# Xinjie-Q/Boosting-NeRV

Hardware: AMD Instinct MI355X
Metric: train frames/sec (higher is better)
Workload: dtype fp32; 1 GPU; NeRV-boost 1.5M (1489577 params, fc_dim 30) train step on a synthetic Bunny-shaped clip 132x3x720x1280: decoder fwd + Fusion10_freq + bwd + fused Adan; frames resident in HBM; global_batch=1, per_gpu_batch=1, parallelism=dp1, hipgraph=True, rccl_ranks=0, collective_in_graph=False

## Files before the change

boosting_nerv_amd/_lib.py:

```python
import ctypes as C
import os

import torch

_HERE = os.path.dirname(os.path.abspath(__file__))
LIB_PATH = os.environ.get("BNERV_LIB") or os.path.join(_HERE, "libbnerv_hip.so")

MAX_DENSE_GROUPS = 40
ADAN_MAX_TENSORS = 48
SFT_CHUNKS = 32
LOSS_STATS = 5
DENSE_DX_CHUNK = 64

ACT_NONE, ACT_RELU, ACT_SIN = 0, 1, 2
IN_PLAIN, IN_AFFINE, IN_GELU_AFFINE, IN_UNSHUFFLE, IN_TANHGRAD = 0, 1, 2, 3, 4
EP_BIAS, EP_BIAS_SIN, EP_BIAS_RES, EP_BIAS_TANH, EP_PLAIN, EP_DGELU, EP_DSIN, EP_BIAS_GELU, EP_DGELU_SAVED = 0, 1, 2, 3, 4, 5, 6, 7, 8
CONV_FAM = ("head1_fwd", "head1_dgrad", "head3", "stem_dgrad", "small", "small96", "wide_bf16", "q4", "generic")
WGRAD_FAM = ("stem", "gemm1x1", "lean", "wide_bf16", "wide_f32", "generic")
PAIR_FORM = ("stem", "q4_lean", "small_wide", "bf16_wide", "head")

_fp = C.c_void_p


class DenseFwdDesc(C.Structure):
# ... 83 lines not shown
    "bnerv_abi_version": (_I, []),
    "bnerv_last_error": (C.c_char_p, []),
    "bnerv_build_arch": (C.c_char_p, []),
    "bnerv_pe_fwd_f32": (_I, [_V, _V, _V, _V, _I, _I]),
    "bnerv_pe_fwd_f64": (_I, [_V, _V, _V, _V, _I, _I]),
    "bnerv_pe_fwd_f32_from_f64": (_I, [_V, _V, _V, _V, _I, _I]),
    "bnerv_dense_grouped_fwd": (_I, [_V, C.POINTER(DenseFwdDesc), _I, _I]),
    "bnerv_time_branch_fwd": (_I, [_V, C.POINTER(TimeBranchDesc), C.POINTER(TimeBranchMlp)]),
    "bnerv_dense_grouped_bwd": (_I, [_V, C.POINTER(DenseBwdDesc), _I, _I]),
    "bnerv_sft_affine_fwd": (_I, [_V, _V, _V, _V, _V, _I, _I, _I]),
    "bnerv_sft_affine_bwd": (_I, [_V, _V, _V, _V, _V, _V, _I, _I, _I]),
    "bnerv_reduce_slabs": (_I, [_V, _V, _I, _I, _V]),
    "bnerv_ctx_create": (_I, [C.POINTER(C.c_void_p)]),
    "bnerv_ctx_destroy": (None, [_V]),
    "bnerv_ctx_scratch_bytes": (_Z, [_V]),
    "bnerv_ctx_reserve": (_I, [_V, _Z]),
    "bnerv_ctx_wplan_record": (_I, [_V]),
    "bnerv_ctx_wplan_freeze": (_I, [_V]),
    "bnerv_ctx_wplan_run": (_I, [_V, _V]),
    "bnerv_ctx_wplan_run_fetch": (_I, [_V, _V, _V, _V, _V, _I, _Z, _V, _V]),
    "bnerv_ctx_wplan_end": (_I, [_V]),
    "bnerv_ctx_wplan_entries": (_I, [_V]),
    "bnerv_reduce_slabs_deferred": (_I, [_V, _V, _V, _I, _I, _V]),
    "bnerv_flush_deferred": (_I, [_V, _V]),
    "bnerv_deferred_pending": (_I, [_V]),
    "bnerv_conv_tiles": (_I, [_I, _I]),
    "bnerv_conv_igemm": (_I, [_V, C.POINTER(ConvDesc)]),
    "bnerv_conv_splitk_ws_bytes": (_Z, [C.POINTER(ConvDesc)]),
    "bnerv_conv_partial_rows": (_I, [C.POINTER(ConvDesc)]),
    "bnerv_conv_family": (_I, [C.POINTER(ConvDesc), C.POINTER(C.c_int)]),
    "bnerv_conv_wgrad_ws_bytes": (_Z, [_I, _I, _I, _I, _I, _I]),
    "bnerv_conv_wgrad_pair": (_I, [_V, C.POINTER(ConvDesc), C.POINTER(WgradDesc)]),
    "bnerv_conv_wgrad_pair_form": (_I, [C.POINTER(ConvDesc), C.POINTER(WgradDesc), C.POINTER(C.c_int)]),
    "bnerv_conv_wgrad": (_I, [_V, C.POINTER(WgradDesc)]),
    "bnerv_conv_wgrad_family": (_I, [C.POINTER(WgradDesc), C.POINTER(C.c_int)]),
    "bnerv_conv5_ws_bytes": (_Z, [_I, _I]),
    "bnerv_conv5_igemm": (_I, [_V, C.POINTER(ConvDesc), _V, _Z]),
    "bnerv_conv5_wgrad_ws_bytes": (_Z, [_I, _I, _I, _I, _I]),
    "bnerv_conv5_wgrad": (_I, [_V, C.POINTER(WgradDesc)]),
    "bnerv_gelu_fwd": (_I, [_V, _V, _V, _V, _Z]),
    "bnerv_mul": (_I, [_V, _V, _V, _V, _Z]),
    "bnerv_cem_ws_bytes": (_Z, [_I, _I]),
    "bnerv_cem_scale_fwd": (_I, [_V, C.POINTER(CemChunk), _V, _V, _Z]),
    "bnerv_cem_scale_bwd": (_I, [_V, C.POINTER(CemChunkBwd), _V, _V, _V, _V, _Z]),
    "bnerv_dense_gemm_fwd": (_I, [_V, _V, _V, _V, _V, _V, _I, _I, _I, _I]),
    "bnerv_dense_gemm_bwd_ws_bytes": (_Z, [_I, _I, _I]),
    "bnerv_dense_gemm_bwd": (_I, [_V, _V, _V, _V, _V, _V, _V, _V, _V, _V, _Z, _I, _I, _I, _I]),
    "bnerv_cnx_mlp_fwd": (_I, [_V, _V, _V, _V, _V, _V, _V, _V, _V, _V, _I, _I, _I]),
    "bnerv_cnx_mlp_bwd": (_I, [_V, _V, _V, _V, _V, _V, _V, _V, _V, _I, _I, _I]),
    "bnerv_cnx_param_grads": (_I, [_V, _V, _V, _V, _V, _V, _V, _V, _V, _I]),
    "bnerv_ans_encode_gaussian": (C.c_long, [_V, _Z, _I, _I, C.c_double, C.c_double, _V, _Z]),
    "bnerv_ans_decode_gaussian": (_I, [_V, _Z, _Z, _I, _I, C.c_double, C.c_double, _V]),
    "bnerv_ans_encode_categorical": (C.c_long, [_V, _Z, _V, _I, _V, _Z]),
    "bnerv_ans_decode_categorical": (_I, [_V, _Z, _Z, _V, _I, _V]),
    "bnerv_dwconv_fwd": (_I, [_V, _V, _V, _V, _V, _I, _I, _I, _I, _I, _I]),
    "bnerv_dwconv_wgrad_ws_bytes": (_Z, [_I, _I, _I, _I, _I]),
    "bnerv_dwconv_wgrad": (_I, [_V, _V, _V, _V, _V, _Z, _I, _I, _I, _I, _I, _V]),
    "bnerv_lncf_fwd": (_I, [_V, _V, _V, _V, _V, _I, _I, _I, _F]),
    "bnerv_lncf_bwd_ws_bytes": (_Z, [_I, _I, _I]),
    "bnerv_lncf_bwd": (_I, [_V, _V, _V, _V, _V, _V, _V, _Z, _I, _I, _I, _F]),
    "bnerv_loss_ws_bytes": (_Z, [_I, _I, _I, _I, _I, _I]),
    "bnerv_fft_prepare": (_I, [_I, _I]),
    "bnerv_loss_fwd_bwd": (_I, [_V, C.POINTER(LossDesc)]),
    "bnerv_msssim": (_I, [_V, _V, _V, _V, _V, _Z, _I, _I, _I, _I]),
    "bnerv_loss_ssim_ws_bytes": (_Z, [_I, _I, _I, _I, _I]),
    "bnerv_loss_ssim_prepare": (_I, [_I, _I]),
# ... 158 lines not shown
```

boosting_nerv_amd/csrc/abi.hip:

```cpp
#include "common.h"
#include <string.h>

namespace { thread_local char g_err[512] = ""; }

int bnerv_set_error(int code, const char* fmt, ...) {
    va_list ap;
    va_start(ap, fmt);
    vsnprintf(g_err, sizeof(g_err), fmt, ap);
    va_end(ap);
    return code;
}

extern "C" int bnerv_abi_version(void) { return BNERV_ABI_VERSION; }
extern "C" const char* bnerv_last_error(void) { return g_err; }
extern "C" const char* bnerv_build_arch(void) { return "gfx950"; }

#include "sidejob.h"
#include <new>
#include <vector>

namespace {
__global__ __launch_bounds__(256) void side_flush_kernel(const SidePack sp) {
    __shared__ float red[256];
    side_slice<SidePack, true>(sp, blockIdx.x, red);
// ... 19 lines not shown
    j.slices = (count + j.epb - 1) / j.epb;
    return j;
}
}

void bnerv_side_push(bnerv_ctx* ctx, hipStream_t st, const void* src, int n_slabs, int count, int ncols, float* out, float* out2, const float* fold_scale, const float* fold_shift) {
    const SideJob j = make_job(src, n_slabs, count, ncols, out, out2, fold_scale, fold_shift);
    if (ctx) { ctx->queue.push_back(j); return; }
    SidePack sp;
    sp.j[0] = j;
    sp.n_jobs = 1;
    sp.n_slices = j.slices;
    hipLaunchKernelGGL(side_flush_kernel, dim3(sp.n_slices), dim3(256), 0, st, sp);
}

void bnerv_side_take(bnerv_ctx* ctx, SidePack* sp, int max_slices) {
    sp->n_jobs = 0;
    sp->n_slices = 0;
    if (!ctx) return;
    std::vector<SideJob>& q = ctx->queue;
    int n = 0;
    size_t i = 0;
    while (i < q.size() && n < SIDE_MAX_JOBS) {
        if (q[i].fs) { ++i; continue; }
        if (sp->n_slices + q[i].slices > max_slices) break;
        sp->j[n] = q[i];
        sp->n_slices += q[i].slices;
        ++n;
        q.erase(q.begin() + (long)i);
    }
    sp->n_jobs = n;
}

int bnerv_side_pending(const bnerv_ctx* ctx) { return ctx ? (int)ctx->queue.size() : 0; }

int bnerv_side_flush(bnerv_ctx* ctx, hipStream_t st) {
    while (ctx && !ctx->queue.empty()) {
        SideFlushPack sp;
        std::vector<SideJob>& q = ctx->queue;
        int n = 0;
        sp.n_slices = 0;
        while (n < (int)q.size() && n < SIDE_FLUSH_JOBS) {
            sp.j[n] = q[n];
            sp.start[n] = sp.n_slices;
            sp.n_slices += q[n].slices;
            ++n;
        }
        for (int k = n; k < SIDE_FLUSH_JOBS; ++k) sp.start[k] = 0x7fffffff;
        sp.n_jobs = n;
        q.erase(q.begin(), q.begin() + n);
        hipLaunchKernelGGL(side_flush_many_kernel, dim3(sp.n_slices), dim3(256), 0, st, sp);
        BNERV_LAUNCH_CHECK("side_flush");
    }
    return BNERV_OK;
}

extern "C" int bnerv_ctx_create(bnerv_ctx** out) {
    BNERV_REQUIRE(out != nullptr, "ctx_create: null output");
    *out = new (std::nothrow) bnerv_ctx();
    return *out ? BNERV_OK : bnerv_set_error(BNERV_E_ARG, "ctx_create: out of memory");
}
extern "C" void bnerv_ctx_destroy(bnerv_ctx* ctx) {
    if (ctx && ctx->scratch) (void)hipFree(ctx->scratch);
    if (ctx) bnerv_wplan_free(ctx);
    delete ctx;
}

extern "C" size_t bnerv_ctx_scratch_bytes(const bnerv_ctx* ctx) { return ctx ? ctx->scratch_bytes : 0; }

// ... 36 lines not shown
```

boosting_nerv_amd/csrc/sidejob.h:

```cpp
#pragma once
#include "common.h"

constexpr int SIDE_MAX_JOBS = 4;

struct SideJob {
    const float* src;
    float* out;
    float* out2;
    int n_slabs, count, ncols;
    int epb;
    int slices;
    const float* fs;
    const float* ft;
};

struct SidePack {
    SideJob j[SIDE_MAX_JOBS];
    int n_jobs, n_slices;
};
constexpr int SIDE_FLUSH_JOBS = 32;
struct SideFlushPack {
    SideJob j[SIDE_FLUSH_JOBS];
    int n_jobs, n_slices;
    int start[SIDE_FLUSH_JOBS];
};

#include <vector>
struct bnerv_ctx {
    std::vector<SideJob> queue;
    void* scratch = nullptr;
    size_t scratch_bytes = 0;
    struct BfWPlan* wplan = nullptr;
};
void bnerv_wplan_free(bnerv_ctx* ctx);
void* bnerv_ctx_scratch(bnerv_ctx* ctx, size_t bytes, hipStream_t st);

void bnerv_side_push(bnerv_ctx* ctx, hipStream_t st, const void* src, int n_slabs, int count, int ncols, float* out, float* out2,
                     const float* fold_scale = nullptr, const float* fold_shift = nullptr);
void bnerv_side_take(bnerv_ctx* ctx, SidePack* sp, int max_slices);
int bnerv_side_flush(bnerv_ctx* ctx, hipStream_t st);
int bnerv_side_pending(const bnerv_ctx* ctx);

template <class Pack>
__device__ __forceinline__ int side_find_job(const Pack& sp, int* s) {
    int j = 0;
    while (j < sp.n_jobs - 1 && *s >= sp.j[j].slices) { *s -= sp.j[j].slices; ++j; }
    return j;
}
template <>
__device__ __forceinline__ int side_find_job<SideFlushPack>(const SideFlushPack& sp, int* s) {
    const int k = (int)(threadIdx.x & 63);
    const int st = k < sp.n_jobs ? sp.start[k < SIDE_FLUSH_JOBS ? k : 0] : 0x7fffffff;
    const unsigned long long m = __ballot(st <= *s);
    const int j = __popcll(m) - 1;
    *s -= __shfl(st, j, 64);
    return __builtin_amdgcn_readfirstlane(j);
}

template <class Pack, bool FOLD = false>
__device__ __forceinline__ void side_slice(const Pack& sp, int s, float* red) {
    const int j = side_find_job(sp, &s);
    const SideJob& job = sp.j[j];
    const int epb = job.epb, lanes = 256 / epb;
    const int e = threadIdx.x % epb, lane = threadIdx.x / epb;
    const int i = s * epb + e;
    const bool fold = FOLD && job.fs != nullptr;
    float acc = 0.f, acc2 = 0.f;
    int fci = 0;
    bool fbias = false;
    if (i < job.count) {
        size_t cnt = (size_t)job.count;
        size_t i0 = (size_t)i, i1 = 0;
        if (fold) {
            const int co = i / job.ncols, n = i - co * job.ncols, rowl = job.ncols + 8;
// ... 58 lines not shown
```

boosting_nerv_amd/csrc/wgrad.hip:

```cpp
#include "common.h"
#include "sidejob.h"
#include "split16.h"
#include "conv4_body.h"
#include "convs_body.h"
#if defined(BNERV_TRACE) || defined(BNERV_TRACE_BW)
static __device__ unsigned long long g_trace_w[1024 * 4 * 8 * 8];
#endif
#ifdef BNERV_TRACE_BW
#define BTRACE(it_, slot) do { if (lane == 0 && blockIdx.x < 1024 && (unsigned)(it_) < 8u) g_trace_w[((blockIdx.x * 4 + wave) * 8 + (it_)) * 8 + (slot)] = __builtin_amdgcn_s_memtime(); } while (0)
#endif
#include "wgrad_bfw_body.h"
#include "route.h"
bool bnerv_stem_wgrad_ok(const bnerv_wgrad_desc& d);
int bnerv_stem_wgrad_launch(hipStream_t st, const bnerv_wgrad_desc& d);
bool bnerv_stem_pair_ok(const bnerv_conv_desc& c, const bnerv_wgrad_desc& d);
int bnerv_stem_pair_launch(hipStream_t st, const bnerv_conv_desc& c, const bnerv_wgrad_desc& d);
int bnerv_wgrad1x1_slabs(const bnerv_wgrad_desc& d);
int bnerv_wgrad1x1_launch(hipStream_t st, const bnerv_wgrad_desc& d);

namespace {
using namespace bnerv_wb;

constexpr int TH = 8, TW = 32;
constexpr int CSG = TH * TW + 2;
// ... 1335 lines not shown
    const bool red_ep = c.ep_mode == BNERV_EP_DGELU_SAVED || c.ep_mode == BNERV_EP_DSIN;
    const int fused_min = fused_env >= 0 ? fused_env : (red_ep ? 1024 : 0);
    if (fused_min > 0 && total_items >= fused_min && total_items >= 8 && c.x == w.g && c.Cin == w.Cout && c.Cout == w.Cin && c.B == w.B &&
        w.g_s == 1 && (w.g_mode == BNERV_IN_PLAIN || w.g_mode == BNERV_IN_UNSHUFFLE)) {
        p.kind = Q4P_SHARED;
        p.grid = p.n_w = total_items < 512 ? (total_items & ~7) : 512;
        const float* raw_aux = c.ep_mode == BNERV_EP_DSIN ? c.aux0 : c.aux1;
        if (red_ep && w.in_mode == BNERV_IN_AFFINE && !switch_off("BNERV_PAIR_FOLD") && c.B == 1 && raw_aux == w.x && w.scale && w.shift && aligned16(w.x) &&
            (size_t)p.grid * w.Cout * (ncols + 8) * sizeof(float) <= w.ws_bytes)
            p.kind = Q4P_FOLD;
        return p;
    }
    p.kind = Q4P_INTERLEAVED;
    p.n_conv = total_items < 768 ? total_items : 768;
    p.n_conv = (p.n_conv + 7) & ~7;
    p.n_w = wlean_blocks(w);
    p.grid = p.n_conv + p.n_w;
    if (total_items >= 2 * PAIR_MIX && p.n_w >= PAIR_MIX) {
        p.n_w = PAIR_MIX; p.n_conv = -PAIR_MIX; p.grid = 2 * PAIR_MIX;
    }
    return p;
}

template <class F>
int q4_pair_modes(const bnerv_conv_desc& c, const bnerv_wgrad_desc& w, F&& f) {
#define BNERV_PAIR_CASE(E, I) if (c.ep_mode == E && w.in_mode == I) return f(mode_c<E>{}, mode_c<I>{});
    BNERV_PAIR_CASE(BNERV_EP_DGELU_SAVED, BNERV_IN_AFFINE)
    BNERV_PAIR_CASE(BNERV_EP_DSIN, BNERV_IN_AFFINE)
    BNERV_PAIR_CASE(BNERV_EP_PLAIN, BNERV_IN_PLAIN)
#undef BNERV_PAIR_CASE
    return -1;
}

template <int EP, int WIN>
int launch_pair(hipStream_t st, bnerv_conv::KArgs& ka, const WArgs& wa, const Q4PairPlan& p) {
    bnerv_q4::q4_prepare(ka);
    SidePack side;
    if (p.kind == Q4P_FOLD) {
        if constexpr ((EP == BNERV_EP_DGELU_SAVED || EP == BNERV_EP_DSIN) && WIN == BNERV_IN_AFFINE) {
            const size_t ldsf = pair_fused_lds_bytes();
            if (const int rc = dyn_lds<&pair_fused_kernel<EP, WIN>>(ldsf, "pair_fused")) return rc;
            const size_t ldsd = pair_fold_lds_bytes();
            if (const int rc = dyn_lds<&pair_fold_kernel<EP>>(ldsd, "pair_fold")) return rc;
            bnerv_side_take(wa.d.ctx, &side, 2 * p.n_w);
            hipLaunchKernelGGL((pair_fold_kernel<EP>), dim3(p.grid), dim3(256), ldsd, st, ka, wa, side);
            BNERV_LAUNCH_CHECK("pair_fold");
            return BNERV_OK;
        }
    }
    if (p.kind != Q4P_INTERLEAVED) {
        const size_t ldsf = pair_fused_lds_bytes();
        if (const int rc = dyn_lds<&pair_fused_kernel<EP, WIN>>(ldsf, "pair_fused")) return rc;
        bnerv_side_take(wa.d.ctx, &side, 2 * p.n_w);
        hipLaunchKernelGGL((pair_fused_kernel<EP, WIN>), dim3(p.grid), dim3(256), ldsf, st, ka, wa, side);
        BNERV_LAUNCH_CHECK("pair_fused");
        return BNERV_OK;
    }
    const int n_grows = wa.d.Cout <= 12 ? 12 : 16;
    size_t lds = bnerv_q4::q4_lds_bytes();
    const size_t lw = wlean_lds_bytes<3>(n_grows);
    if (lw > lds) lds = lw;
    if (const int rc = dyn_lds<&conv_wgrad_pair_kernel<EP, WIN>>(lds, "conv_wgrad_pair")) return rc;
    bnerv_side_take(wa.d.ctx, &side, 2 * p.n_w);
    hipLaunchKernelGGL((conv_wgrad_pair_kernel<EP, WIN>), dim3(p.grid), dim3(256), lds, st, ka, wa, n_grows, p.n_conv, side, PAIR_PAT);
    BNERV_LAUNCH_CHECK("conv_wgrad_pair");
    return BNERV_OK;
}

struct WideRoleArgs { int slots, ngn, ngm; };
template <int IN, int GM2, int MTW, int NTW>
struct WideRole {
    static __device__ __forceinline__ void run(const WArgs& wa, const WideRoleArgs& r, const SidePack& side, int vb, int vgrid) { wgrad_wide_body<IN, GM2, MTW, NTW>(wa, r.slots, side, vb, vgrid); }
    static size_t lds(const WArgs& wa) { return wgrad_wide_lds_bytes<MTW, NTW>(wa.d.Cout); }
};
template <int IN, int SP, int MTW, int GM2>
struct BfwRole {
    static __device__ __forceinline__ void run(const WArgs& wa, const WideRoleArgs& r, const SidePack& side, int vb, int vgrid) { wgrad_bfw_body<IN, SP, MTW, GM2>(wa, r.slots, r.ngn, r.ngm, side, vb, vgrid); }
    static size_t lds(const WArgs&) { return wgrad_bfw_lds_bytes<SP, MTW>(); }
};
template <class WR, int CIN, int CEP, int CNQ>
__global__ __launch_bounds__(256, 2) void small_pair_kernel(const bnerv_convs::SArgs sa, const WArgs wa, const WideRoleArgs r, const int n_c, const int n_c8,
                                                            const int c_tiles, const int c_groups, const SidePack side) {
    const int b = (int)blockIdx.x;
    if (b < n_c8) {
        if (b >= n_c) return;
        const int q = b / c_tiles;
        bnerv_convs::conv_small_body<CIN, CEP, CNQ>(sa, b - q * c_tiles, q % c_groups, q / c_groups);
    } else {
        WR::run(wa, r, side, b - n_c8, (int)gridDim.x - n_c8);
    }
}
template <class WR, int CIN, int CEP, int CNQ>
int launch_small_pair(hipStream_t st, const bnerv_convs::SArgs& sa, const WArgs& wa, const WideRoleArgs& r, int n_w) {
    size_t lds = bnerv_convs::convs_lds_bytes<CNQ>();
    const size_t lw = WR::lds(wa);
    if (lw > lds) lds = lw;
    if (const int rc = dyn_lds<&small_pair_kernel<WR, CIN, CEP, CNQ>>(lds, "small_pair")) return rc;
    const int c_tiles = sa.tiles_x * sa.tiles_y, c_groups = cdiv(sa.d.Cout, 16);
    const int n_c = c_tiles * c_groups * sa.d.B, n_c8 = (n_c + 7) & ~7;
    SidePack side;
    bnerv_side_take(wa.d.ctx, &side, 2 * n_w);
    hipLaunchKernelGGL((small_pair_kernel<WR, CIN, CEP, CNQ>), dim3(n_c8 + n_w), dim3(256), lds, st, sa, wa, r, n_c, n_c8, c_tiles, c_groups, side);
    BNERV_LAUNCH_CHECK("small_pair");
    return BNERV_OK;
}

template <class T> struct type_c { using type = T; };
template <class F>
int small_pair_modes(const bnerv_conv_desc& c, const bnerv_wgrad_desc& w, const WRoute& wr, F&& f) {
    const int cnq = bnerv_convs_nq(c);
    const bool up = w.g_s == 2 && w.in_mode == BNERV_IN_PLAIN && w.g_mode == BNERV_IN_UNSHUFFLE;
    const bool tat = w.g_s == 1 && w.in_mode == BNERV_IN_AFFINE && w.g_mode != BNERV_IN_TANHGRAD;
#define BNERV_SP(WR, I, E, Q) if (c.in_mode == I && c.ep_mode == E && cnq == Q) return f(type_c<WR>{}, mode_c<I>{}, mode_c<E>{}, mode_c<Q>{});
    if (wr.family == BNERV_WGRAD_FAM_WIDE_BF16 && split_wide_mode() == (int)SP_BF16X6) {
        if (up && wr.bw.mtw == 2) { using WR = BfwRole<BNERV_IN_PLAIN, SP_BF16X6, 2, 1>; BNERV_SP(WR, BNERV_IN_UNSHUFFLE, BNERV_EP_PLAIN, 8) BNERV_SP(WR, BNERV_IN_UNSHUFFLE, BNERV_EP_PLAIN, 16) }
        if (up && wr.bw.mtw == 3) { using WR = BfwRole<BNERV_IN_PLAIN, SP_BF16X6, 3, 1>; BNERV_SP(WR, BNERV_IN_UNSHUFFLE, BNERV_EP_PLAIN, 16) }
        if (tat && wr.bw.mtw == 2) { using WR = BfwRole<BNERV_IN_AFFINE, SP_BF16X6, 2, 0>; BNERV_SP(WR, BNERV_IN_PLAIN, BNERV_EP_DGELU_SAVED, 8) BNERV_SP(WR, BNERV_IN_PLAIN, BNERV_EP_DSIN, 8) }
    }
    if (wr.family == BNERV_WGRAD_FAM_WIDE_F32 && wr.wide.mtw == 1 && wr.wide.ntw == 8 && tat) {
        using WR = WideRole<BNERV_IN_AFFINE, 0, 1, 8>;
        BNERV_SP(WR, BNERV_IN_PLAIN, BNERV_EP_DGELU_SAVED, 4) BNERV_SP(WR, BNERV_IN_PLAIN, BNERV_EP_DSIN, 4)
    }
#undef BNERV_SP
    return -1;
}

bool small_pair_ok(const bnerv_conv_desc& c, int cvec, const bnerv_wgrad_desc& w, const WRoute& wr) {
    if (!bnerv_convs_ok(c, cvec) || bnerv_convs_nq(c) == 24) return false;
    if (c.ep_mode == BNERV_EP_PLAIN && bnerv_conv_splitk_ws_bytes(&c) != 0) return false;
    if (!(w.k == 3 && w.B == c.B && w.H == c.H && w.W == c.W && w.defer_finish && w.ctx && w.ctx == c.ctx)) return false;
    return small_pair_modes(c, w, wr, [](auto...) { return 0; }) == 0;
}

int small_pair_launch(hipStream_t st, const bnerv_conv_desc& c, const WArgs& wa, const WRoute& wr) {
    const bnerv_convs::SArgs sa = bnerv_convs_sargs(c);
    const bool bf = wr.family == BNERV_WGRAD_FAM_WIDE_BF16;
    const WideRoleArgs r = bf ? WideRoleArgs{wr.bw.slots, wr.bw.ngroups_n, wr.bw.ngroups_m} : WideRoleArgs{wr.wide.slots, 0, 0};
    const int n_w = bf ? 8 * wr.bw.slots * wr.bw.ngroups_n * wr.bw.ngroups_m : 8 * wr.wide.slots * wr.wide.ngroups * wr.wide.mgroups;
    return small_pair_modes(c, wa.d, wr, [&](auto role, auto in, auto ep, auto nq) {
        return launch_small_pair<typename decltype(role)::type, decltype(in)::value, decltype(ep)::value, decltype(nq)::value>(st, sa, wa, r, n_w);
    });
}
}

constexpr int HB_KMAX = 4, HB_CMAX = 16;
struct HeadBwdArgs { const float* g; const float* img; const float* x; const float* w; float* dx; float* slab; int B, K, C, transposed; size_t HW; int nq; };
template <int K, int C>
__global__ __launch_bounds__(256) void head1x1_bwd_kernel(const HeadBwdArgs a) {
    __shared__ float s_w[HB_KMAX * HB_CMAX];
    __shared__ float s_red[4][HB_KMAX * (HB_CMAX + 1)];
    const int tid = threadIdx.x, lane = tid & 63, wave = tid >> 6;
    if (tid < K * C) {
        const int k = tid / C, c = tid - k * C;
        s_w[k * HB_CMAX + c] = a.transposed ? a.w[k * C + c] : a.w[c * K + k];
    }
    if (lane < K * (C + 1)) s_red[wave][(lane / (C + 1)) * (HB_CMAX + 1) + lane % (C + 1)] = 0.f;
    __syncthreads();
    const int total = a.B * a.nq;
    const int rounds = (total + (int)gridDim.x * 256 - 1) / ((int)gridDim.x * 256);
#pragma unroll 1
    for (int it = 0; it < rounds; ++it) {
        const int q = (it * (int)gridDim.x + (int)blockIdx.x) * 256 + tid;
        const bool live = q < total;
        const int b = live ? q / a.nq : 0, qq = live ? q - b * a.nq : 0;
        f32x4 dy[K];
#pragma unroll
        for (int k = 0; k < K; ++k) {
            const size_t o = ((size_t)b * K + k) * a.HW + (size_t)qq * 4;
            const f32x4 v = *reinterpret_cast<const f32x4*>(a.g + o), im = *reinterpret_cast<const f32x4*>(a.img + o);
#pragma unroll
            for (int e = 0; e < 4; ++e) { const float t = 2.0f * im[e] - 1.0f; dy[k][e] = live ? v[e] * 0.5f * (1.0f - t * t) : 0.f; }
        }
        f32x4 xv[C];
// ... 91 lines not shown
    if (w.Cin <= 0 || w.Cout <= 0) return p;
    if (w.ws_bytes < bnerv_conv_wgrad_ws_bytes(w.B, w.Cin, w.Cout, w.H, w.W, w.k)) {
        p.rc = BNERV_E_WS;
        return p;
    }
    p.cvec = conv_vec_ok(c);
    p.wvec = wgrad_vec(w, false);
    p.wr = wgrad_route(w, p.wvec, BNERV_WGRAD_FAM_LEAN);
    if (c.in_mode == BNERV_IN_PLAIN && w.g_s == 1 && p.wr.family == BNERV_WGRAD_FAM_LEAN && bnerv_q4::q4_shape_ok(bnerv_conv_kargs(c, p.cvec)) &&
        q4_pair_modes(c, w, [](auto, auto) { return 0; }) == 0) {
        p.form = BNERV_PAIR_Q4_LEAN;
        p.q4 = q4_pair_plan(c, w);
        p.n_slabs = p.q4.n_w;
        p.fold = p.q4.kind == Q4P_FOLD;
        return p;
    }
    if (!no_bf16 && p.wr.family == BNERV_WGRAD_FAM_WIDE_BF16 && split_wide_mode() == (int)SP_BF16X6) {
        p.bf = bnerv_convbf_pair_plan(c, p.cvec, w, p.wr.bw);
        if (p.bf.take) {
            p.form = BNERV_PAIR_BF16_WIDE;
            p.n_slabs = 8 * p.bf.slots;
            return p;
        }
    }
    if (small_pair_ok(c, p.cvec, w, p.wr)) {
        p.form = BNERV_PAIR_SMALL_WIDE;
        p.th = BNERV_CONVS_TH;
        p.tw = BNERV_CONVS_TW;
        p.n_slabs = p.wr.n_slabs;
    }
    return p;
}

PairPlan pair_plan(const bnerv_conv_desc& c, const bnerv_wgrad_desc& w, bool no_bf16 = false) {
    PairPlan p = pair_form(c, w, no_bf16);
    const bool sums = c.ep_mode == BNERV_EP_DGELU || c.ep_mode == BNERV_EP_DSIN || c.ep_mode == BNERV_EP_DGELU_SAVED;
    if (p.form != BNERV_PAIR_NONE && sums && cdiv(c.H, p.th) * cdiv(c.W, p.tw) != bnerv_conv_partial_rows(&c)) {
        p.form = BNERV_PAIR_NONE;
        p.rc = 1;
    }
    return p;
}

bnerv_conv_desc pair_conv_desc(const bnerv_conv_desc& cd) {
    bnerv_conv_desc c = cd;
    if (c.in_mode == BNERV_IN_UNSHUFFLE && c.in_s == 1) c.in_mode = BNERV_IN_PLAIN;
    return c;
}
}

extern "C" int bnerv_conv_wgrad_pair_form(const bnerv_conv_desc* cdp, const bnerv_wgrad_desc* wdp, int* conv_rows) {
    if (conv_rows) *conv_rows = 0;
    if (!cdp || !wdp || cdp->H <= 0 || cdp->W <= 0 || cdp->B <= 0 || cdp->Cin <= 0 || cdp->Cout <= 0) return BNERV_PAIR_NONE;
    const bnerv_conv_desc c = pair_conv_desc(*cdp);
    const PairPlan p = pair_plan(c, *wdp);
    if (conv_rows && p.form != BNERV_PAIR_NONE) *conv_rows = cdiv(c.H, p.th) * cdiv(c.W, p.tw);
    return p.form;
}

extern "C" int bnerv_conv_wgrad_pair(void* stream, const bnerv_conv_desc* cdp, const bnerv_wgrad_desc* wdp) {
    BNERV_REQUIRE(cdp != nullptr && wdp != nullptr, "conv_wgrad_pair: null descriptor");
    const bnerv_conv_desc c = pair_conv_desc(*cdp);
    const bnerv_wgrad_desc& w = *wdp;
    hipStream_t st = reinterpret_cast<hipStream_t>(stream);
    PairPlan p = pair_plan(c, w);
    for (;;) {
        int rc = p.rc;
        switch (p.form) {
        case BNERV_PAIR_HEAD:
            if ((rc = head_pair_launch(st, c, w, p.n_slabs)) == BNERV_OK) bnerv_side_push(w.ctx, st, w.ws, p.n_slabs, w.Cout * (w.Cin + 1), w.Cin + 1, w.dw, w.db);
            return rc;
        case BNERV_PAIR_STEM:
            if ((rc = bnerv_stem_pair_launch(st, c, w)) == BNERV_OK) bnerv_side_push(c.ctx, st, c.partial, p.n_slabs, c.B * c.Cout * c.H * c.W, 0, c.out, nullptr);
            return rc;
        case BNERV_PAIR_NONE: return rc == BNERV_E_WS ? bnerv_set_error(rc, "conv_wgrad_pair: weight-gradient workspace too small") : rc;
        default: break;
        }
        const WArgs wa = wgrad_args(w, p.wr, p.wvec);
        if (p.form == BNERV_PAIR_Q4_LEAN) {
            bnerv_conv::KArgs ka = bnerv_conv_kargs(c, p.cvec);
            rc = q4_pair_modes(c, w, [&](auto ep, auto in) { return launch_pair<decltype(ep)::value, decltype(in)::value>(st, ka, wa, p.q4); });
        } else if (p.form == BNERV_PAIR_BF16_WIDE) {
            rc = bnerv_convbf_pair_launch(st, c, wa, p.wr.bw, p.bf);
            if (rc == BNERV_DECLINED) {
                p = pair_plan(c, w, true);
                continue;
            }
        } else {
            rc = small_pair_launch(st, c, wa, p.wr);
        }
        if (rc != BNERV_OK) return rc;
        if (p.fold) bnerv_side_push(w.ctx, st, wa.slab, p.n_slabs, w.Cout * wa.ncols, wa.ncols, w.dw, w.db, w.scale, w.shift);
        else bnerv_side_push(w.ctx, st, wa.slab, p.n_slabs, w.Cout * wa.ncols, wa.ncols, w.dw, w.db);
        return BNERV_OK;
    }
}
```

boosting_nerv_amd/csrc/wgrad_bfw_body.h:

```cpp
#pragma once
#include "common.h"
#include "sidejob.h"
#include "split16.h"
#ifndef BTRACE
#define BTRACE(it_, slot) do {} while (0)
#endif

namespace bnerv_wb {

struct WArgs {
    bnerv_wgrad_desc d;
    float* slab;
    int tiles_x, tiles_y, n_mgroups, n_ngroups, ncols;
    int vec;
};

typedef int i32x4 __attribute__((ext_vector_type(4)));
constexpr unsigned OOB = 0x80000000u;

__device__ __forceinline__ __amdgpu_buffer_rsrc_t make_rsrc(const float* p, unsigned shift_bytes, unsigned bytes) {
    return __builtin_amdgcn_make_buffer_rsrc(reinterpret_cast<void*>(reinterpret_cast<uintptr_t>(p) - shift_bytes), 0, (int)bytes, 0x00020000);
}
__device__ __forceinline__ f32x4 bload(__amdgpu_buffer_rsrc_t r, unsigned voff, unsigned soff) {
    return __builtin_bit_cast(f32x4, __builtin_amdgcn_raw_buffer_load_b128(r, (int)voff, (int)soff, 0));
}

struct LTile { int b, ty, tx; };

constexpr int BW_TH = 4, BW_NTW = 8, BW_NPL = (BW_NTW * 16 + 7) / 9 + 1;
constexpr int BW_ROW = 64, BW_PLANE = 6 * BW_ROW + 32, BW_COPY = BW_NPL * BW_PLANE + 192, BW_CONST = 4 * BW_ROW;
constexpr int BW_PIECE = 3 * BW_COPY + 2 * BW_CONST;

template <int IN, int SP, int MTW, int GM2>
__device__ __forceinline__ void wgrad_bfw_body(const WArgs& wa, const int slots, const int ngroups_n, const int ngroups_m, const SidePack& side, const int vb, const int vgrid) {
    constexpr int NS = Split<SP>::NS;
    constexpr bool AFF = (IN == BNERV_IN_AFFINE);
    constexpr int PIECE = BW_PIECE;
    const bnerv_wgrad_desc& d = wa.d;
    extern __shared__ __attribute__((aligned(16))) float smem[];
    char* s_a = reinterpret_cast<char*>(smem);
    float* s_aff = reinterpret_cast<float*>(s_a + NS * PIECE);
    const int tid = threadIdx.x, lane = tid & 63;
    const int wave = __builtin_amdgcn_readfirstlane(tid >> 6);
    const int li = lane & 15, kq = lane >> 4;
    const int Cin = d.Cin, Cout = d.Cout, H = d.H, W = d.W;
    const int nW = Cin * 9;
    const int tiles_x = (W + 31) >> 5, tiles_y = (H + BW_TH - 1) / BW_TH;

// ... 303 lines not shown
```

boosting_nerv_amd/ops.py:

```python
import ctypes as C
import os

import torch
import torch.nn.functional as F

from . import _lib as L


def _ws(nbytes, device):
    return torch.empty(max(int(nbytes), 16), dtype=torch.uint8, device=device)


_STREAM_CTX = object()
_SUMS_EP = (L.EP_DGELU, L.EP_DSIN, L.EP_DGELU_SAVED)


def _conv_desc(x, w, bias, out, *, B, Cin, Cout, H, W, k, in_mode, ep_mode, in_s=1, out_s=1, transposed=0, out2=None,
               aux0=None, aux1=None, aux2=None, scale=None, shift=None, partial=None, ctx=_STREAM_CTX):
    return L.ConvDesc(L.ptr(x), L.ptr(w), L.ptr(bias), L.ptr(out), L.ptr(out2), L.ptr(aux0), L.ptr(aux1), L.ptr(aux2),
                      L.ptr(scale), L.ptr(shift), L.ptr(partial), B, Cin, Cout, H, W, k, in_mode, ep_mode, in_s, out_s,
                      transposed, w.shape[0], w.shape[1], L.ctx().handle if ctx is _STREAM_CTX else ctx)


def _wgrad_desc(x, g, dw, db, ws, ws_bytes, *, B, Cin, Cout, H, W, k, in_mode, g_mode, g_s=1, gaux=None, scale=None, shift=None,
# ... 40 lines not shown
def _wgrad(x, g, dw, db, *, B, Cin, Cout, H, W, k, in_mode, g_mode, g_s=1, gaux=None, scale=None, shift=None, defer=False):
    lib = L.load()
    nbytes = lib.bnerv_conv_wgrad_ws_bytes(B, Cin, Cout, H, W, k)
    ws = _ws(nbytes, x.device)
    d = _wgrad_desc(x, g, dw, db, ws, nbytes, B=B, Cin=Cin, Cout=Cout, H=H, W=W, k=k, in_mode=in_mode, g_mode=g_mode, g_s=g_s, gaux=gaux,
                    scale=scale, shift=shift, defer=defer)
    L.check(lib.bnerv_conv_wgrad(L.stream(), C.byref(d)), "bnerv_conv_wgrad")
    if defer:
        L.ctx().keep.append(ws)


def _wgrad_conv_pair(wg, cv):
    lib = L.load()
    dev = wg["x"].device
    nbytes = lib.bnerv_conv_wgrad_ws_bytes(wg["B"], wg["Cin"], wg["Cout"], wg["H"], wg["W"], wg["k"])
    ws = _ws(nbytes, dev)
    wd = _wgrad_desc(ws=ws, ws_bytes=nbytes, **{**wg, "defer": True})
    cd = _conv_desc(**cv)
    red = cv["ep_mode"] in _SUMS_EP
    skw = None
    if red:
        part, rows = _sums_partial(cd, dev)
    elif cv["ep_mode"] == L.EP_PLAIN:
        skw = _splitk_ws(cd, dev)
    rc = lib.bnerv_conv_wgrad_pair(L.stream(), C.byref(cd), C.byref(wd))
    if rc == 1:
        L.check(lib.bnerv_conv_wgrad(L.stream(), C.byref(wd)), "bnerv_conv_wgrad")
        L.check(lib.bnerv_conv_igemm(L.stream(), C.byref(cd)), "bnerv_conv_igemm")
    else:
        L.check(rc, "bnerv_conv_wgrad_pair")
    dx_queued = rc != 1 and skw is not None
    if dx_queued:
        L.ctx().keep.append(skw)
    L.ctx().keep.append(ws)
    return (_reduced_sums(part, rows, cd, dev, True) if red else None), dx_queued


def _reduce_slabs(slabs, n_slabs, count, out, defer=False):
    if defer:
        c = L.ctx()
        L.check(L.load().bnerv_reduce_slabs_deferred(c.handle, L.stream(), L.ptr(slabs), n_slabs, count, L.ptr(out)), "bnerv_reduce_slabs_deferred")
        c.keep.append(slabs)
        return
    L.check(L.load().bnerv_reduce_slabs(L.stream(), L.ptr(slabs), n_slabs, count, L.ptr(out)), "bnerv_reduce_slabs")


_lazy = []


def _flush_deferred():
    c = L.ctx()
    L.check(L.load().bnerv_flush_deferred(c.handle, L.stream()), "bnerv_flush_deferred")
    c.keep.clear()
    c.dx_queued = False


def _end_block(dx_queued=False):
    if _lazy and (not dx_queued or _lazy[-1]):
        if dx_queued:
            L.ctx().dx_queued = True
        return
    _flush_deferred()


def _enter_backward(reads_sums=False):
    c = L.ctx(create=False)
# ... 899 lines not shown
```

include/bnerv.h:

```cpp
#ifndef BNERV_H
#define BNERV_H

#include <stddef.h>
#include <stdint.h>

#ifdef __cplusplus
extern "C" {
#endif

#define BNERV_ABI_VERSION 9

#define BNERV_OK 0
#define BNERV_E_ARG (-1)
#define BNERV_E_LAUNCH (-2)
#define BNERV_E_WS (-3)

int bnerv_abi_version(void);
const char* bnerv_last_error(void);
const char* bnerv_build_arch(void);

int bnerv_pe_fwd_f32(void* stream, const float* pos, const float* bases, float* out, int N, int L);
int bnerv_pe_fwd_f64(void* stream, const double* pos, const float* bases, float* out, int N, int L);
int bnerv_pe_fwd_f32_from_f64(void* stream, const double* pos, const float* bases, float* out, int N, int L);

// ... 194 lines not shown
    const float* pred;
    const float* target;
    float* grad;
    float* loss_out;
    float* stats_out;
    void* ws;
    size_t ws_bytes;
    int B, C, H, W;
    float c_l1, c_l2, c_ms, c_fft;
} bnerv_loss_desc;

size_t bnerv_loss_ws_bytes(int B, int C, int H, int W, int use_ms, int use_fft);
int bnerv_fft_prepare(int H, int W);
int bnerv_loss_fwd_bwd(void* stream, const bnerv_loss_desc* d);
int bnerv_msssim(void* stream, const float* x, const float* y, float* out, void* ws, size_t ws_bytes, int B, int C, int H, int W);
size_t bnerv_loss_ssim_ws_bytes(int B, int C, int H, int W, int use_fft);
int bnerv_loss_ssim_prepare(int H, int W);
int bnerv_loss_ssim_fwd_bwd(void* stream, const bnerv_loss_desc* d, float c_ssim);
int bnerv_ssim(void* stream, const float* x, const float* y, float* out, void* ws, size_t ws_bytes, int B, int C, int H, int W);
int bnerv_tanh_grad_blocks(int HW);
int bnerv_tanh_grad(void* stream, const float* g, const float* img, float* gt, float* part, int B, int C, int HW);

size_t bnerv_psnr_ws_bytes(int B, int C, int H, int W);
int bnerv_psnr(void* stream, const float* out, const float* gt, float* psnr, void* ws, size_t ws_bytes, int B, int C, int H, int W);

int bnerv_conv_wgrad_pair(void* stream, const bnerv_conv_desc* conv, const bnerv_wgrad_desc* wgrad);
#define BNERV_PAIR_NONE (-1)
#define BNERV_PAIR_STEM 0
#define BNERV_PAIR_Q4_LEAN 1
#define BNERV_PAIR_SMALL_WIDE 2
#define BNERV_PAIR_BF16_WIDE 3
#define BNERV_PAIR_HEAD 4
int bnerv_conv_wgrad_pair_form(const bnerv_conv_desc* conv, const bnerv_wgrad_desc* wgrad, int* conv_rows);

#define BNERV_ADAN_MAX_TENSORS 48
typedef struct {
    float* p[BNERV_ADAN_MAX_TENSORS];
    const float* g[BNERV_ADAN_MAX_TENSORS];
    float* exp_avg[BNERV_ADAN_MAX_TENSORS];
    float* exp_avg_sq[BNERV_ADAN_MAX_TENSORS];
    float* exp_avg_diff[BNERV_ADAN_MAX_TENSORS];
    float* neg_pre_grad[BNERV_ADAN_MAX_TENSORS];
    int n[BNERV_ADAN_MAX_TENSORS];
    int n_tensors;
} bnerv_adan_chunk;

typedef struct {
    float beta1, beta2, beta3;
    float eps, weight_decay;
    float clip_global_grad_norm;
    int no_prox;
    const float* sched_dev;
} bnerv_adan_hyper;

int bnerv_adan_multi_tensor(void* stream, const bnerv_adan_chunk* chunk, const bnerv_adan_hyper* h);

typedef struct {
    float* p;
    const float* g;
    float* exp_avg;
    float* exp_avg_sq;
    float* exp_avg_diff;
    float* neg_pre_grad;
    int n;
    int bstart;
} bnerv_adan_entry;
// ... 23 lines not shown
```

Before: 680.1 frames/s.

## Defer small-layer weight-gradient work into a batched drain kernel

For small-resolution Q4-lean and small-wide conv/wgrad pairs, the conv (dgrad) part now launches alone and the weight-gradient role is queued on the context. At side-flush time all queued wgrad roles run in one multi-job drain kernel, and their slab reductions are then pushed onto the side queue. The goal is to cut per-layer launch count and let small wgrad jobs fill the GPU together instead of sharing blocks with small conv grids. In exchange, input tensors must stay alive until the drain, and the drain kernel uses the largest LDS footprint of the batched roles, which can reduce its occupancy.

```diff
diff --git a/boosting_nerv_amd/_lib.py b/boosting_nerv_amd/_lib.py
--- a/boosting_nerv_amd/_lib.py
+++ b/boosting_nerv_amd/_lib.py
@@ -139,6 +139,9 @@
     "bnerv_conv_wgrad_ws_bytes": (_Z, [_I, _I, _I, _I, _I, _I]),
     "bnerv_conv_wgrad_pair": (_I, [_V, C.POINTER(ConvDesc), C.POINTER(WgradDesc)]),
     "bnerv_conv_wgrad_pair_form": (_I, [C.POINTER(ConvDesc), C.POINTER(WgradDesc), C.POINTER(C.c_int)]),
+    "bnerv_conv_wgrad_pair_deferred_ws_bytes": (_Z, [C.POINTER(ConvDesc), C.POINTER(WgradDesc)]),
+    "bnerv_wgrad_drain": (_I, [_V, _V]),
+    "bnerv_ctx_wgrad_queue": (_I, [_V, _I]),
     "bnerv_conv_wgrad": (_I, [_V, C.POINTER(WgradDesc)]),
     "bnerv_conv_wgrad_family": (_I, [C.POINTER(WgradDesc), C.POINTER(C.c_int)]),
     "bnerv_conv5_ws_bytes": (_Z, [_I, _I]),
diff --git a/boosting_nerv_amd/csrc/abi.hip b/boosting_nerv_amd/csrc/abi.hip
--- a/boosting_nerv_amd/csrc/abi.hip
+++ b/boosting_nerv_amd/csrc/abi.hip
@@ -75,9 +75,10 @@
     sp->n_jobs = n;
 }
 
-int bnerv_side_pending(const bnerv_ctx* ctx) { return ctx ? (int)ctx->queue.size() : 0; }
+int bnerv_side_pending(const bnerv_ctx* ctx) { return ctx ? (int)(ctx->queue.size() + ctx->wqueue.size()) : 0; }
 
 int bnerv_side_flush(bnerv_ctx* ctx, hipStream_t st) {
+    if (const int rc = bnerv_wgrad_drain_queue(ctx, st)) return rc;
     while (ctx && !ctx->queue.empty()) {
         SideFlushPack sp;
         std::vector<SideJob>& q = ctx->queue;
diff --git a/boosting_nerv_amd/csrc/sidejob.h b/boosting_nerv_amd/csrc/sidejob.h
--- a/boosting_nerv_amd/csrc/sidejob.h
+++ b/boosting_nerv_amd/csrc/sidejob.h
@@ -25,9 +25,37 @@
     int start[SIDE_FLUSH_JOBS];
 };
 
+namespace bnerv_wb {
+struct WArgs {
+    bnerv_wgrad_desc d;
+    float* slab;
+    int tiles_x, tiles_y, n_mgroups, n_ngroups, ncols;
+    int vec;
+};
+}
+struct WQRole {
+    bnerv_wb::WArgs wa;
+    int kind;
+    int p0, p1, p2;
+    int vgrid;
+};
+struct WQJob {
+    WQRole r;
+    int n_slabs;
+    size_t lds;
+};
+constexpr int WQ_MAX_JOBS = 16;
+struct WQPack {
+    WQRole j[WQ_MAX_JOBS];
+    int start[WQ_MAX_JOBS];
+    int n_jobs;
+};
+
 #include <vector>
 struct bnerv_ctx {
     std::vector<SideJob> queue;
+    std::vector<WQJob> wqueue;
+    bool wq_on = true;
     void* scratch = nullptr;
     size_t scratch_bytes = 0;
     struct BfWPlan* wplan = nullptr;
@@ -40,6 +68,7 @@
 void bnerv_side_take(bnerv_ctx* ctx, SidePack* sp, int max_slices);
 int bnerv_side_flush(bnerv_ctx* ctx, hipStream_t st);
 int bnerv_side_pending(const bnerv_ctx* ctx);
+int bnerv_wgrad_drain_queue(bnerv_ctx* ctx, hipStream_t st);
 
 template <class Pack>
 __device__ __forceinline__ int side_find_job(const Pack& sp, int* s) {
diff --git a/boosting_nerv_amd/csrc/wgrad.hip b/boosting_nerv_amd/csrc/wgrad.hip
--- a/boosting_nerv_amd/csrc/wgrad.hip
+++ b/boosting_nerv_amd/csrc/wgrad.hip
@@ -1391,8 +1391,78 @@
     return -1;
 }
 
+struct WideRoleArgs { int slots, ngn, ngm; };
+template <int IN, int GM2, int MTW, int NTW>
+struct WideRole {
+    static __device__ __forceinline__ void run(const WArgs& wa, const WideRoleArgs& r, const SidePack& side, int vb, int vgrid) { wgrad_wide_body<IN, GM2, MTW, NTW>(wa, r.slots, side, vb, vgrid); }
+    static size_t lds(const WArgs& wa) { return wgrad_wide_lds_bytes<MTW, NTW>(wa.d.Cout); }
+};
+template <int IN, int SP, int MTW, int GM2>
+struct BfwRole {
+    static __device__ __forceinline__ void run(const WArgs& wa, const WideRoleArgs& r, const SidePack& side, int vb, int vgrid) { wgrad_bfw_body<IN, SP, MTW, GM2>(wa, r.slots, r.ngn, r.ngm, side, vb, vgrid); }
+    static size_t lds(const WArgs&) { return wgrad_bfw_lds_bytes<SP, MTW>(); }
+};
+template <int WIN>
+struct LeanRole {
+    static __device__ __forceinline__ void run(const WArgs& wa, const WideRoleArgs& r, const SidePack& side, int vb, int vgrid) { wgrad_lean_body<3, WIN, 0>(wa, r.slots, side, vb, vgrid); }
+    static size_t lds(const WArgs& wa) { return wlean_lds_bytes<3>(wa.d.Cout <= 12 ? 12 : 16); }
+};
+template <class T> struct type_c { using type = T; };
+
+template <class WR>
+constexpr int wq_kind() {
+    if (std::is_same<WR, LeanRole<BNERV_IN_AFFINE>>::value) return 0;
+    if (std::is_same<WR, LeanRole<BNERV_IN_PLAIN>>::value) return 1;
+    if (std::is_same<WR, WideRole<BNERV_IN_AFFINE, 0, 1, 8>>::value) return 2;
+    if (std::is_same<WR, BfwRole<BNERV_IN_PLAIN, SP_BF16X6, 2, 1>>::value) return 3;
+    if (std::is_same<WR, BfwRole<BNERV_IN_PLAIN, SP_BF16X6, 3, 1>>::value) return 4;
+    if (std::is_same<WR, BfwRole<BNERV_IN_AFFINE, SP_BF16X6, 2, 0>>::value) return 5;
+    return -1;
+}
+__global__ __launch_bounds__(256, 2) void wgrad_drain_kernel(const WQPack qp) {
+    const int k = (int)(threadIdx.x & 63);
+    const int st = k < qp.n_jobs ? qp.start[k < WQ_MAX_JOBS ? k : 0] : 0x7fffffff;
+    const unsigned long long m = __ballot(st <= (int)blockIdx.x);
+    const int j = __builtin_amdgcn_readfirstlane(__popcll(m) - 1);
+    const WQRole& q = qp.j[j];
+    const int vb = (int)blockIdx.x - qp.start[j];
+    const WideRoleArgs r{q.p0, q.p1, q.p2};
+    SidePack none;
+    none.n_jobs = 0; none.n_slices = 0;
+    switch (q.kind) {
+    case 0: LeanRole<BNERV_IN_AFFINE>::run(q.wa, r, none, vb, q.vgrid); break;
+    case 1: LeanRole<BNERV_IN_PLAIN>::run(q.wa, r, none, vb, q.vgrid); break;
+    case 2: WideRole<BNERV_IN_AFFINE, 0, 1, 8>::run(q.wa, r, none, vb, q.vgrid); break;
+    case 3: BfwRole<BNERV_IN_PLAIN, SP_BF16X6, 2, 1>::run(q.wa, r, none, vb, q.vgrid); break;
+    case 4: BfwRole<BNERV_IN_PLAIN, SP_BF16X6, 3, 1>::run(q.wa, r, none, vb, q.vgrid); break;
+    default: BfwRole<BNERV_IN_AFFINE, SP_BF16X6, 2, 0>::run(q.wa, r, none, vb, q.vgrid); break;
+    }
+}
+void wq_push(const WArgs& wa, int kind, const WideRoleArgs& r, int vgrid, int n_slabs, size_t lds) {
+    WQJob j;
+    j.r.wa = wa;
+    j.r.kind = kind;
+    j.r.p0 = r.slots; j.r.p1 = r.ngn; j.r.p2 = r.ngm;
+    j.r.vgrid = vgrid;
+    j.n_slabs = n_slabs;
+    j.lds = lds;
+    wa.d.ctx->wqueue.push_back(j);
+}
+
+template <int EP>
+__global__ __launch_bounds__(256, 3) void q4_role_kernel(const bnerv_conv::KArgs ka) {
+    SidePack none;
+    none.n_jobs = 0; none.n_slices = 0;
+    bnerv_q4::conv_q4_body<BNERV_IN_PLAIN, EP>(ka, none, (int)blockIdx.x, (int)gridDim.x);
+}
+template <int CIN, int CEP, int CNQ>
+__global__ __launch_bounds__(256, 4) void small_role_kernel(const bnerv_convs::SArgs sa, const int c_tiles, const int c_groups) {
+    const int b = (int)blockIdx.x, q = b / c_tiles;
+    bnerv_convs::conv_small_body<CIN, CEP, CNQ>(sa, b - q * c_tiles, q % c_groups, q / c_groups);
+}
+
 template <int EP, int WIN>
-int launch_pair(hipStream_t st, bnerv_conv::KArgs& ka, const WArgs& wa, const Q4PairPlan& p) {
+int launch_pair(hipStream_t st, bnerv_conv::KArgs& ka, const WArgs& wa, const Q4PairPlan& p, bool defer) {
     bnerv_q4::q4_prepare(ka);
     SidePack side;
     if (p.kind == Q4P_FOLD) {
@@ -1418,6 +1488,14 @@
     const int n_grows = wa.d.Cout <= 12 ? 12 : 16;
     size_t lds = bnerv_q4::q4_lds_bytes();
     const size_t lw = wlean_lds_bytes<3>(n_grows);
+    if (defer) {
+        static_assert(wq_kind<LeanRole<WIN>>() >= 0, "a role of form 1 the drain kernel lacks");
+        if (const int rc = dyn_lds<&q4_role_kernel<EP>>(lds, "q4_role")) return rc;
+        hipLaunchKernelGGL((q4_role_kernel<EP>), dim3(p.n_conv), dim3(256), lds, st, ka);
+        BNERV_LAUNCH_CHECK("q4_role");
+        wq_push(wa, wq_kind<LeanRole<WIN>>(), WideRoleArgs{n_grows, 0, 0}, p.n_w, p.n_w, lw);
+        return BNERV_OK;
+    }
     if (lw > lds) lds = lw;
     if (const int rc = dyn_lds<&conv_wgrad_pair_kernel<EP, WIN>>(lds, "conv_wgrad_pair")) return rc;
     bnerv_side_take(wa.d.ctx, &side, 2 * p.n_w);
@@ -1426,17 +1504,6 @@
     return BNERV_OK;
 }
 
-struct WideRoleArgs { int slots, ngn, ngm; };
-template <int IN, int GM2, int MTW, int NTW>
-struct WideRole {
-    static __device__ __forceinline__ void run(const WArgs& wa, const WideRoleArgs& r, const SidePack& side, int vb, int vgrid) { wgrad_wide_body<IN, GM2, MTW, NTW>(wa, r.slots, side, vb, vgrid); }
-    static size_t lds(const WArgs& wa) { return wgrad_wide_lds_bytes<MTW, NTW>(wa.d.Cout); }
-};
-template <int IN, int SP, int MTW, int GM2>
-struct BfwRole {
-    static __device__ __forceinline__ void run(const WArgs& wa, const WideRoleArgs& r, const SidePack& side, int vb, int vgrid) { wgrad_bfw_body<IN, SP, MTW, GM2>(wa, r.slots, r.ngn, r.ngm, side, vb, vgrid); }
-    static size_t lds(const WArgs&) { return wgrad_bfw_lds_bytes<SP, MTW>(); }
-};
 template <class WR, int CIN, int CEP, int CNQ>
 __global__ __launch_bounds__(256, 2) void small_pair_kernel(const bnerv_convs::SArgs sa, const WArgs wa, const WideRoleArgs r, const int n_c, const int n_c8,
                                                             const int c_tiles, const int c_groups, const SidePack side) {
@@ -1450,13 +1517,21 @@
     }
 }
 template <class WR, int CIN, int CEP, int CNQ>
-int launch_small_pair(hipStream_t st, const bnerv_convs::SArgs& sa, const WArgs& wa, const WideRoleArgs& r, int n_w) {
+int launch_small_pair(hipStream_t st, const bnerv_convs::SArgs& sa, const WArgs& wa, const WideRoleArgs& r, int n_w, int n_slabs, bool defer) {
     size_t lds = bnerv_convs::convs_lds_bytes<CNQ>();
     const size_t lw = WR::lds(wa);
+    const int c_tiles = sa.tiles_x * sa.tiles_y, c_groups = cdiv(sa.d.Cout, 16);
+    const int n_c = c_tiles * c_groups * sa.d.B, n_c8 = (n_c + 7) & ~7;
+    if (defer) {
+        static_assert(wq_kind<WR>() >= 0, "a role of form 2 the drain kernel lacks");
+        if (const int rc = dyn_lds<&small_role_kernel<CIN, CEP, CNQ>>(lds, "small_role")) return rc;
+        hipLaunchKernelGGL((small_role_kernel<CIN, CEP, CNQ>), dim3(n_c), dim3(256), lds, st, sa, c_tiles, c_groups);
+        BNERV_LAUNCH_CHECK("small_role");
+        wq_push(wa, wq_kind<WR>(), r, n_w, n_slabs, lw);
+        return BNERV_OK;
+    }
     if (lw > lds) lds = lw;
     if (const int rc = dyn_lds<&small_pair_kernel<WR, CIN, CEP, CNQ>>(lds, "small_pair")) return rc;
-    const int c_tiles = sa.tiles_x * sa.tiles_y, c_groups = cdiv(sa.d.Cout, 16);
-    const int n_c = c_tiles * c_groups * sa.d.B, n_c8 = (n_c + 7) & ~7;
     SidePack side;
     bnerv_side_take(wa.d.ctx, &side, 2 * n_w);
     hipLaunchKernelGGL((small_pair_kernel<WR, CIN, CEP, CNQ>), dim3(n_c8 + n_w), dim3(256), lds, st, sa, wa, r, n_c, n_c8, c_tiles, c_groups, side);
@@ -1464,7 +1539,6 @@
     return BNERV_OK;
 }
 
-template <class T> struct type_c { using type = T; };
 template <class F>
 int small_pair_modes(const bnerv_conv_desc& c, const bnerv_wgrad_desc& w, const WRoute& wr, F&& f) {
     const int cnq = bnerv_convs_nq(c);
@@ -1491,13 +1565,13 @@
     return small_pair_modes(c, w, wr, [](auto...) { return 0; }) == 0;
 }
 
-int small_pair_launch(hipStream_t st, const bnerv_conv_desc& c, const WArgs& wa, const WRoute& wr) {
+int small_pair_launch(hipStream_t st, const bnerv_conv_desc& c, const WArgs& wa, const WRoute& wr, bool defer) {
     const bnerv_convs::SArgs sa = bnerv_convs_sargs(c);
     const bool bf = wr.family == BNERV_WGRAD_FAM_WIDE_BF16;
     const WideRoleArgs r = bf ? WideRoleArgs{wr.bw.slots, wr.bw.ngroups_n, wr.bw.ngroups_m} : WideRoleArgs{wr.wide.slots, 0, 0};
     const int n_w = bf ? 8 * wr.bw.slots * wr.bw.ngroups_n * wr.bw.ngroups_m : 8 * wr.wide.slots * wr.wide.ngroups * wr.wide.mgroups;
     return small_pair_modes(c, wa.d, wr, [&](auto role, auto in, auto ep, auto nq) {
-        return launch_small_pair<typename decltype(role)::type, decltype(in)::value, decltype(ep)::value, decltype(nq)::value>(st, sa, wa, r, n_w);
+        return launch_small_pair<typename decltype(role)::type, decltype(in)::value, decltype(ep)::value, decltype(nq)::value>(st, sa, wa, r, n_w, wr.n_slabs, defer);
     });
 }
 }
@@ -1655,6 +1729,17 @@
     return p;
 }
 
+constexpr size_t WQ_MAX_PIXELS = 180 * 320;
+bool pair_wgrad_deferred(const PairPlan& p, const bnerv_conv_desc& c, const bnerv_wgrad_desc& w) {
+    if (!w.ctx || !w.defer_finish) return false;
+    if ((size_t)c.H * c.W > WQ_MAX_PIXELS) return false;
+    if (p.form == BNERV_PAIR_Q4_LEAN)
+        return p.q4.kind == Q4P_INTERLEAVED && p.q4.n_conv > 0 && c.B * cdiv(c.W, bnerv_conv::TW) * cdiv(c.H, bnerv_conv::TH) <= 768;
+    if (p.form == BNERV_PAIR_SMALL_WIDE)
+        return c.B * cdiv(c.W, BNERV_CONVS_TW) * cdiv(c.H, BNERV_CONVS_TH) * cdiv(c.Cout, 16) <= 1024;
+    return false;
+}
+
 PairPlan pair_plan(const bnerv_conv_desc& c, const bnerv_wgrad_desc& w, bool no_bf16 = false) {
     PairPlan p = pair_form(c, w, no_bf16);
     const bool sums = c.ep_mode == BNERV_EP_DGELU || c.ep_mode == BNERV_EP_DSIN || c.ep_mode == BNERV_EP_DGELU_SAVED;
@@ -1680,6 +1765,48 @@
     if (conv_rows && p.form != BNERV_PAIR_NONE) *conv_rows = cdiv(c.H, p.th) * cdiv(c.W, p.tw);
     return p.form;
 }
+
+extern "C" size_t bnerv_conv_wgrad_pair_deferred_ws_bytes(const bnerv_conv_desc* cdp, const bnerv_wgrad_desc* wdp) {
+    if (!cdp || !wdp || cdp->H <= 0 || cdp->W <= 0 || cdp->B <= 0 || cdp->Cin <= 0 || cdp->Cout <= 0) return 0;
+    const bnerv_conv_desc c = pair_conv_desc(*cdp);
+    const PairPlan p = pair_plan(c, *wdp);
+    return pair_wgrad_deferred(p, c, *wdp) ? (size_t)p.n_slabs * wdp->Cout * (wdp->Cin * 9 + 1) * sizeof(float) : 0;
+}
+
+int bnerv_wgrad_drain_queue(bnerv_ctx* ctx, hipStream_t st) {
+    while (ctx && !ctx->wqueue.empty()) {
+        std::vector<WQJob>& q = ctx->wqueue;
+        WQPack qp;
+        int n = 0, blocks = 0;
+        size_t lds = 0;
+        while (n < (int)q.size() && n < WQ_MAX_JOBS) {
+            qp.j[n] = q[n].r;
+            qp.start[n] = blocks;
+            blocks += q[n].r.vgrid;
+            if (q[n].lds > lds) lds = q[n].lds;
+            ++n;
+        }
+        for (int k = n; k < WQ_MAX_JOBS; ++k) qp.start[k] = 0x7fffffff;
+        qp.n_jobs = n;
+        const std::vector<WQJob> done(q.begin(), q.begin() + n);
+        q.erase(q.begin(), q.begin() + n);
+        if (const int rc = dyn_lds<&wgrad_drain_kernel>(lds, "wgrad_drain")) return rc;
+        hipLaunchKernelGGL(wgrad_drain_kernel, dim3(blocks), dim3(256), lds, st, qp);
+        BNERV_LAUNCH_CHECK("wgrad_drain");
+        for (const WQJob& j : done) {
+            const bnerv_wgrad_desc& w = j.r.wa.d;
+            bnerv_side_push(ctx, st, j.r.wa.slab, j.n_slabs, w.Cout * j.r.wa.ncols, j.r.wa.ncols, w.dw, w.db);
+        }
+    }
+    return BNERV_OK;
+}
+extern "C" int bnerv_ctx_wgrad_queue(bnerv_ctx* ctx, int on) {
+    if (!ctx) return 0;
+    const int was = ctx->wq_on ? 1 : 0;
+    ctx->wq_on = on != 0;
+    return was;
+}
+extern "C" int bnerv_wgrad_drain(bnerv_ctx* ctx, void* stream) { return bnerv_wgrad_drain_queue(ctx, reinterpret_cast<hipStream_t>(stream)); }
 
 extern "C" int bnerv_conv_wgrad_pair(void* stream, const bnerv_conv_desc* cdp, const bnerv_wgrad_desc* wdp) {
     BNERV_REQUIRE(cdp != nullptr && wdp != nullptr, "conv_wgrad_pair: null descriptor");
@@ -1700,9 +1827,10 @@
         default: break;
         }
         const WArgs wa = wgrad_args(w, p.wr, p.wvec);
+        const bool defer = pair_wgrad_deferred(p, c, w) && w.ctx->wq_on;
         if (p.form == BNERV_PAIR_Q4_LEAN) {
             bnerv_conv::KArgs ka = bnerv_conv_kargs(c, p.cvec);
-            rc = q4_pair_modes(c, w, [&](auto ep, auto in) { return launch_pair<decltype(ep)::value, decltype(in)::value>(st, ka, wa, p.q4); });
+            rc = q4_pair_modes(c, w, [&](auto ep, auto in) { return launch_pair<decltype(ep)::value, decltype(in)::value>(st, ka, wa, p.q4, defer); });
         } else if (p.form == BNERV_PAIR_BF16_WIDE) {
             rc = bnerv_convbf_pair_launch(st, c, wa, p.wr.bw, p.bf);
             if (rc == BNERV_DECLINED) {
@@ -1710,9 +1838,9 @@
                 continue;
             }
         } else {
-            rc = small_pair_launch(st, c, wa, p.wr);
-        }
-        if (rc != BNERV_OK) return rc;
+            rc = small_pair_launch(st, c, wa, p.wr, defer);
+        }
+        if (rc != BNERV_OK || defer) return rc;
         if (p.fold) bnerv_side_push(w.ctx, st, wa.slab, p.n_slabs, w.Cout * wa.ncols, wa.ncols, w.dw, w.db, w.scale, w.shift);
         else bnerv_side_push(w.ctx, st, wa.slab, p.n_slabs, w.Cout * wa.ncols, wa.ncols, w.dw, w.db);
         return BNERV_OK;
diff --git a/boosting_nerv_amd/csrc/wgrad_bfw_body.h b/boosting_nerv_amd/csrc/wgrad_bfw_body.h
--- a/boosting_nerv_amd/csrc/wgrad_bfw_body.h
+++ b/boosting_nerv_amd/csrc/wgrad_bfw_body.h
@@ -7,13 +7,6 @@
 #endif
 
 namespace bnerv_wb {
-
-struct WArgs {
-    bnerv_wgrad_desc d;
-    float* slab;
-    int tiles_x, tiles_y, n_mgroups, n_ngroups, ncols;
-    int vec;
-};
 
 typedef int i32x4 __attribute__((ext_vector_type(4)));
 constexpr unsigned OOB = 0x80000000u;
diff --git a/boosting_nerv_amd/ops.py b/boosting_nerv_amd/ops.py
--- a/boosting_nerv_amd/ops.py
+++ b/boosting_nerv_amd/ops.py
@@ -96,6 +96,8 @@
     dx_queued = rc != 1 and skw is not None
     if dx_queued:
         L.ctx().keep.append(skw)
+    if rc != 1 and lib.bnerv_conv_wgrad_pair_deferred_ws_bytes(C.byref(cd), C.byref(wd)):
+        ws = (ws, wg["x"], wg["g"], wg.get("gaux"), wg.get("scale"), wg.get("shift"))
     L.ctx().keep.append(ws)
     return (_reduced_sums(part, rows, cd, dev, True) if red else None), dx_queued
 
diff --git a/include/bnerv.h b/include/bnerv.h
--- a/include/bnerv.h
+++ b/include/bnerv.h
@@ -250,6 +250,9 @@
 #define BNERV_PAIR_BF16_WIDE 3
 #define BNERV_PAIR_HEAD 4
 int bnerv_conv_wgrad_pair_form(const bnerv_conv_desc* conv, const bnerv_wgrad_desc* wgrad, int* conv_rows);
+size_t bnerv_conv_wgrad_pair_deferred_ws_bytes(const bnerv_conv_desc* conv, const bnerv_wgrad_desc* wgrad);
+int bnerv_ctx_wgrad_queue(bnerv_ctx* ctx, int on);
+int bnerv_wgrad_drain(bnerv_ctx* ctx, void* stream);
 
 #define BNERV_ADAN_MAX_TENSORS 48
 typedef struct {
```

Result: no change. 684.9 frames/s, median of 6 (+0.7%).
